# zalgo3/zfista

Hardware: AMD Instinct MI355X
Metric: fista_iterations_per_sec_n1e8_per_gpu_shard (higher is better)
Workload: dtype f64

## Files before the change

zfista_amd/_lib.py:

```python
from __future__ import annotations

import ctypes as C
import os
import subprocess

import numpy as np

_HERE = os.path.dirname(os.path.abspath(__file__))
CSRC = os.path.join(_HERE, "csrc")
LIB_PATH = os.environ.get("ZF_LIB_PATH") or os.path.join(CSRC, "libzfista_hip.so")

ZF_OK = 0
ZF_RUNNING, ZF_CONVERGED, ZF_MAXITER, ZF_BACKTRACK_FAILED = 0, 1, 2, 3
ZF_PROBLEM_DIAG_QUAD_L1, ZF_PROBLEM_LEAST_SQUARES_L1, ZF_PROBLEM_BLUR_HAAR_L1 = 1, 2, 3
ZF_PROBLEM_SPARSE_LS_L1 = 4
ZF_PROBLEM_LOGISTIC_L1, ZF_PROBLEM_SPARSE_LOGISTIC_L1 = 5, 6
ZF_MO_GENERIC, ZF_MO_JOS1, ZF_MO_FDS = 0, 1, 2
ZF_PACK_LEN, ZF_TRACE_COLS, ZF_RING = 8, 8, 1024
ZF_MAX_SUB_ITERS = 16
ZF_MAX_LAG = 2 * ZF_MAX_SUB_ITERS - 2
ZF_PEND_FLUSH = -1
TR_ERR, TR_F, TR_LR, TR_FUN, TR_TRIALS, TR_FX, TR_GX, TR_FY = range(8)
PK_FY, PK_DOT, PK_SS, PK_GX, PK_FX, PK_ERR = range(6)
PK_DF = 7
ZF_ACCEPT_REFERENCE, ZF_ACCEPT_RESOLVED, ZF_ACCEPT_REMAINDER = 0, 1, 2
ACCEPT_MODES = {"reference": ZF_ACCEPT_REFERENCE, "resolved": ZF_ACCEPT_RESOLVED, "remainder": ZF_ACCEPT_REMAINDER}


class HipUnavailable(RuntimeError):
    """The HIP engine cannot be used (library not built, or no GPU)."""


class ZfError(RuntimeError):
    """A libzfista_hip call returned a negative status."""


# ... 219 lines not shown
    lib = load()
    n = C.c_int(0)
    rc = lib.zf_device_count(C.byref(n))
    if rc != ZF_OK or n.value < 1:
        raise HipUnavailable(
            "no usable GPU: " + lib.zf_last_error().decode(errors="replace")
            + " - zfista_amd runs its solver arithmetic on MI355X only (no CPU fallback)."
        )
    return lib


ENV_SWITCHES = ("ZF_SPECULATE", "ZF_LS_SMALL", "ZF_GEMV_MFMA", "ZF_TILES_PER_WG", "ZF_SUB_ITERS",
                "ZF_COMM", "ZF_MO_COMM", "ZF_MO_LAUNCH_AHEAD", "ZF_MO_SPIN_LIMIT", "ZF_RCCL_LIB", "ZF_DUAL_SOLVER",
                "ZF_FORCE_SPLIT", "ZF_LIB_PATH", "ZF_BENCH_BACKEND",
                "ZF_RUNAHEAD", "ZF_RUNAHEAD_SPIN_LIMIT", "ZF_PASS_SEQ_START", "ZF_AHEAD",
                "ZF_AHEAD_UNSHARDED", "ZF_ACCEPT", "ZF_OP_SEPARABLE", "ZF_OP_FUSE_PROX", "ZF_OP_PERSIST", "ZF_RUNAHEAD_SHARDED")


def env_overrides() -> dict:
    return {k: os.environ[k] for k in ENV_SWITCHES if k in os.environ}


def ptr(a: np.ndarray) -> int:
    return a.ctypes.data
```

zfista_amd/csrc/zf_common.h:

```cpp
#pragma once
#include <hip/hip_runtime.h>
#include <stdint.h>
#include <stdio.h>
#include <string.h>

#include "../../include/zfista_hip.h"

extern thread_local char zf_errbuf[512];
static inline int zf_fail(int code, const char* fmt, const char* a = "", const char* b = "") {
    snprintf(zf_errbuf, sizeof(zf_errbuf), fmt, a, b);
    return code;
}
#define ZF_HIP(expr)                                                                   \
    do {                                                                               \
        hipError_t _e = (expr);                                                        \
        if (_e != hipSuccess) return zf_fail(ZF_ERR_HIP, "%s: %s", #expr, hipGetErrorString(_e)); \
    } while (0)
#define ZF_REQUIRE(cond, msg)                                  \
    do {                                                       \
        if (!(cond)) return zf_fail(ZF_ERR_ARG, "%s%s", msg);  \
    } while (0)

struct zf_env {
    bool speculate;
    int pass_seq_start;
    int sub_iters;
    bool runahead;
    int tiles_per_wg;
    unsigned runahead_spin;
    int runahead_sharded;
    bool ahead;
    bool ahead_unsharded;
    bool gemv_mfma;
    bool ls_small;
    bool op_separable;
    bool op_fuse_prox;
    bool op_persist;
    long long mo_spin_limit;
};
zf_env zf_env_read();

constexpr int ZF_BLOCK = 256;
constexpr int ZF_MAX_GRID = 2048;
constexpr int ZF_WAVES = ZF_BLOCK / 64;

static inline int zf_grid_for(int64_t items_per_thread_units) {
    int64_t blocks = (items_per_thread_units + ZF_BLOCK - 1) / ZF_BLOCK;
    if (blocks < 1) blocks = 1;
    if (blocks > ZF_MAX_GRID) blocks = ZF_MAX_GRID;
    return (int)blocks;
}

// ... 107 lines not shown
```

zfista_amd/csrc/zf_decide.h:

```cpp
#pragma once
#include <math.h>
#include <stddef.h>
#include <stdint.h>

#include "../../include/zfista_hip.h"

#if defined(__HIPCC__)
#define ZF_HD __host__ __device__
#else
#define ZF_HD
#endif

enum { ZF_PK_FY = 0, ZF_PK_DOT = 1, ZF_PK_SS = 2, ZF_PK_GX = 3, ZF_PK_FX = 4, ZF_PK_ERR = 5, ZF_PK_DF = 7 };
enum { ZF_TR_ERR = 0, ZF_TR_F = 1, ZF_TR_LR = 2, ZF_TR_FUN = 3, ZF_TR_TRIALS = 4,
       ZF_TR_FX = 5, ZF_TR_GX = 6, ZF_TR_FY = 7 };

ZF_HD inline void zf_reduce_packs(const double* packs, int world, int stride, double* out) {
    for (int k = 0; k < ZF_PACK_LEN; ++k) out[k] = packs[k];
    for (int r = 1; r < world; ++r) {
        const double* p = packs + (int64_t)r * stride;
        for (int k = 0; k < ZF_PACK_LEN; ++k) {
            if (k == ZF_PK_ERR) out[k] = (p[k] > out[k] || p[k] != p[k]) ? p[k] : out[k];
            else out[k] = out[k] + p[k];
        }
    }
}

ZF_HD inline void zf_free_bufs(int cur, int prev, int ring, int* first, int* second) {
    int f[2] = {-1, -1}, m = 0;
    if (ring >= 5) {
// ... 2 lines not shown
            if (i != prev) f[m++] = i;
        }
    } else {
        for (int i = 0; i < ring && m < 2; ++i)
            if (i != cur && i != prev) f[m++] = i;
    }
    *first = f[0];
    *second = (m > 1) ? f[1] : f[0];
}

ZF_HD inline int zf_fresh_len(const zf_control* c) {
    if (c->pend_status != 0) return 0;
    const int sub = c->sub_iters > 0 ? c->sub_iters : 1;
    const int64_t left = c->max_iter - c->nit;
    int64_t n = sub >= 16 ? sub / 2 : sub;
    if (c->lag == 0) {
        if (left >= 2 * (int64_t)sub || left == sub) return sub;
        n = left > sub ? (left + 1) / 2 : left;
    }
    const int64_t cap = (int64_t)(2 * sub - 1) - c->lag;
    if (n > cap) n = cap;
    if (n > left) n = left;
    if (n < 1) n = 1;
    return (int)n;
}

ZF_HD inline double zf_pack_stamp(const zf_control* c) {
    return (double)(((c->total_trials + 1) << 6) | ((int64_t)(c->lag & 31) << 1) | (c->pend_status != 0 ? 1 : 0));
}

typedef struct zf_trial_eval {
// ... 115 lines not shown
    const int sub = ctl->sub_iters > 0 ? ctl->sub_iters : 1;
    const int ring = ctl->ring_size > 0 ? ctl->ring_size : 3;
    const int stride = sub * ZF_PACK_LEN;
    const int lag = ctl->lag;
    zf_control c = *ctl;
    if (ctl->pend_status != 0) {
        if (lag > 0) zf_commit_chain(&c, ctl->cur, ctl->prev, ring, lag);
        c.lag = 0;
        if (c.pend_status > 0) c.status = c.pend_status;
        c.pend_status = 0;
        zf_resolve_beta(&c, beta_ring);
        zf_store_head(ctl, &c);
        return;
    }
    const int nf = zf_fresh_len(ctl);
    int accepted = 0;
    for (int j = 0; j < nf; ++j) {
        const int64_t before = c.nit;
        const double lr_used = c.lr;
        const bool go = zf_decide_step(&c, packs + j * ZF_PACK_LEN, trace, beta_ring, stride, pre ? pre + j : nullptr);
        if (c.nit > before) {
            if (lag + accepted < ZF_MAX_LAG) ctl->lag_lr[lag + accepted] = lr_used;
            accepted += 1;
        }
        if (!go) break;
    }
    if (accepted == nf) {
        zf_commit_chain(&c, ctl->cur, ctl->prev, ring, lag + nf);
        c.lag = 0;
    } else {
        c.lag = lag + accepted;
        if (c.status != ZF_RUNNING && c.lag > 0) {
            c.pend_status = c.status;
            c.status = ZF_RUNNING;
        }
    }
    zf_resolve_beta(&c, beta_ring);
    zf_store_head(ctl, &c);
}

#if defined(__HIPCC__)
__device__ __forceinline__ void zf_decide_pass_wave(zf_control* ctl, const double* packs,
// ... 16 lines not shown
```

zfista_amd/csrc/zf_kernels_step.h:

```cpp
#pragma once
#include <type_traits>

#include "zf_common.h"
#include "zf_decide.h"

constexpr int ZF_NPART = 6;

struct zf_elem_acc {
    double fy, dot, ss, l1, fx, mx;
};

template <bool NESTEROV, bool BOX, bool RES = false>
__device__ __forceinline__ double zf_elem_diag(double xk, double xo, double d, double c, double beta,
                                               double lr, double tau, double lo, double hi,
                                               zf_elem_acc& a) {
    double y = xk;
    if (NESTEROV) y = xk + beta * (xk - xo);
    const double r = y - c;
    const double grad = d * r;
    a.fy = __builtin_fma(grad, r, a.fy);
    const double v = y - lr * grad;
    double xn = zf_soft_threshold_nn(v, tau);
    if (BOX) xn = zf_clip(xn, lo, hi);
    const double dx = xn - y;
// ... 172 lines not shown
    int decide;
    double* trace;
    int pass_seq;
    int fb_on, fb_part, fb_len;
    unsigned long long* ra_word;
    unsigned* ra_flags;
    int ra_wait;
    int ra_need;
    unsigned ra_spin;
    zf_pass_head ra_head;
    unsigned* ra_stats;
    double head_stamp;
    int head_nf;
    int fin_grid;
    int accept_mode;
};

ZF_HD inline int zf_log_shape(int lag, int nf, int passes) { return (nf & 31) | ((lag & 31) << 5) | ((passes & 63) << 10); }

struct zf_finalize_args {
    const double* blk_part;
    int nblocks;
    int sub_iters;
    double* slice_part;
    unsigned* cnt;
    double scale[ZF_NPART];
    const double* f_y_ext;
    const double* f_x_ext;
    const double* r_ext;
    int contribute_f;
// ... 409 lines not shown
__device__ __forceinline__ double zf_readlane_f64(double v, int i) {
    const long long b = __double_as_longlong(v);
    const unsigned lo = (unsigned)__builtin_amdgcn_readlane((int)(unsigned)b, i);
    const unsigned hi = (unsigned)__builtin_amdgcn_readlane((int)(unsigned)(b >> 32), i);
    return __longlong_as_double((long long)(((unsigned long long)hi << 32) | lo));
}
__device__ __forceinline__ zf_pass_head zf_head_of(const zf_control* c) {
    zf_pass_head h;
    h.cur = c->cur;
    h.prev = c->prev;
    h.ring = c->ring_size;
    h.lr = c->lr;
    h.beta_next = c->beta_next;
    h.nit = c->nit;
    return h;
}

template <bool GRAD_INLINE, bool NESTEROV, bool BOX, bool NT, int S, int MODE, bool HIST, int SP = S, bool COH = false, bool RES = false>
__device__ __forceinline__ double zf_trial_body(const zf_step_args& A, double* lds, const zf_pass_head& HD, const int lag,
                                                const int nf, zf_d2* stage = nullptr) {
    constexpr bool FULL = (MODE == 0);
    static_assert(!RES || GRAD_INLINE, "resolved differences f(x+) - f(y): the separable problem");
    static_assert(!COH || (FULL && !HIST && GRAD_INLINE && SP >= 16 && ZF_S16_GLDS != 0),
                  "coherent iterate traffic: branch-free chains of a 16-chain solver through the DMA pipeline");
    constexpr bool GLDS = COH || zf_uses_glds<S, MODE, HIST, GRAD_INLINE, SP>();
    const unsigned tidx = threadIdx.x;
    constexpr bool FRESH_FULL = (MODE <= 1);
    const int cur = HD.cur;
    const int prev = HD.prev;
    const int ring = HD.ring;
// ... 276 lines not shown
                    o = a;
                    a = r;
                    if (HIST) A.hist[((nit + j + 1) % A.hist_cap) * A.hist_stride + e] = a;
                }
            }
            if constexpr (COH) {
                __hip_atomic_store(out_last + e, a, __ATOMIC_RELAXED, __HIP_MEMORY_SCOPE_AGENT);
                __hip_atomic_store(out_prev + e, o, __ATOMIC_RELAXED, __HIP_MEMORY_SCOPE_AGENT);
            } else {
                out_last[e] = a;
                if (S > 1 && (FRESH_FULL || ntr >= 2)) out_prev[e] = o;
            }
        }
    }

    constexpr int RS = S + (S > 1 ? (S & 1) : 0);
    constexpr int H = zf_chain_h(RS);
    constexpr int NQ = S * ZF_NPART;
    const int lane = tidx & 63, wave = tidx >> 6;
    double sums[5 * RS], maxs[RS];
#pragma unroll
    for (int j = 0; j < RS; ++j) {
        if (j < S) {
            sums[j * 5 + 0] = acc[j].fy;
            sums[j * 5 + 1] = acc[j].dot;
            sums[j * 5 + 2] = acc[j].ss;
            sums[j * 5 + 3] = acc[j].l1;
            sums[j * 5 + 4] = acc[j].fx;
            maxs[j] = acc[j].mx;
        } else {
#pragma unroll
            for (int k = 0; k < 5; ++k) sums[j * 5 + k] = 0.0;
            maxs[j] = 0.0;
        }
    }
    zf_wave_reduce_multi<5 * RS, H, false>(sums, lane);
    zf_wave_reduce_multi<RS, H, true>(maxs, lane);
    if ((lane & ((64 >> H) - 1)) == 0) {
#pragma unroll
        for (int q = 0; q < ((5 * RS) >> H); ++q) {
            const int idx = zf_wave_reduce_multi_index<5 * RS, H>(q, lane);
            if (idx / 5 < S) lds[wave * NQ + (idx / 5) * ZF_NPART + idx % 5] = sums[q];
        }
#pragma unroll
        for (int q = 0; q < (RS >> H); ++q) {
            const int tr = zf_wave_reduce_multi_index<RS, H>(q, lane);
            if (tr < S) lds[wave * NQ + tr * ZF_NPART + 5] = maxs[q];
        }
    }
    __syncthreads();
    double v = 0.0;
    if (tidx < NQ) {
        const int t = tidx;
        v = lds[t];
#pragma unroll
        for (int w = 1; w < ZF_WAVES; ++w) v = (t % ZF_NPART == 5) ? fmax(v, lds[w * NQ + t]) : v + lds[w * NQ + t];
    }
    return v;
}

template <int SP>
__device__ __forceinline__ void zf_pass_finish(const zf_step_args& A, const double v) {
    if (A.fin_mode == 0) {
        if (threadIdx.x < SP * ZF_NPART) A.blk_part[(int64_t)threadIdx.x * gridDim.x + blockIdx.x] = v;
// ... 147 lines not shown
    const int go = A.ra_wait == 0 ? 1 : __builtin_amdgcn_readfirstlane(s_go);
    if (go == 0) {
        if (b == 0 && threadIdx.x == 0) __hip_atomic_fetch_add(A.ra_stats + 1, 1u, __ATOMIC_RELAXED, __HIP_MEMORY_SCOPE_AGENT);
        return;
    }
    const bool run = go == 1;
    HD.beta_next = NESTEROV ? zf_uniform_f64(A.beta_ring[HD.nit % ZF_RING]) : 0.0;
    double v = 0.0;
    if (run) v = zf_trial_body<true, NESTEROV, BOX, NT, LEN, 0, false, S, true, RES>(A, lds, HD, 0, LEN, stage);
    zf_step_args T = A;
    T.ctl = A.ctl_rw;
    T.ctl_rw = &s_ctl;
    zf_pass_tail<S, true, LEN>(T, v);
}

template <bool GRAD_INLINE, bool BOX>
__global__ __launch_bounds__(ZF_BLOCK) void zf_eval_kernel(const double* __restrict__ x,
                                                           const double* __restrict__ d,
                                                           const double* __restrict__ c, double lo,
                                                           double hi, int64_t n, double* partials) {
    __shared__ double lds[ZF_WAVES * 3];
    double f = 0.0, l1 = 0.0, viol = 0.0;
    const int64_t stride = (int64_t)gridDim.x * ZF_BLOCK;
    for (int64_t i = (int64_t)blockIdx.x * ZF_BLOCK + threadIdx.x; i < n; i += stride) {
        const double xv = x[i];
        if (GRAD_INLINE) {
            const double r = xv - c[i];
            f += d[i] * (r * r);
        }
        l1 += fabs(xv);
// ... 35 lines not shown
```

zfista_amd/csrc/zf_solver.hip:

```cpp
#include <algorithm>
#include <cstring>
#include <map>
#include <mutex>
#include <new>
#include <tuple>
#include <vector>

#include "zf_common.h"
#include "zf_decide.h"
#include "zf_kernels_gemv.h"
#include "zf_kernels_ls_small.h"
#include "zf_kernels_op.h"
#include "zf_spmv.h"
#include "zf_kernels_loss.h"
#include "zf_kernels_step.h"
#include "zf_trial_launch.h"

thread_local char zf_errbuf[512] = "";

__global__ __launch_bounds__(ZF_BLOCK) void zf_sum_parts_kernel(const zf_control* ctl, const double* __restrict__ s_all,
                                                                int world, int64_t m, zf_ring3 sr, int slot) {
    int idx = 0;
    if (slot >= 0) {
        if (ctl->status != ZF_RUNNING) return;
// ... 199 lines not shown
    double* blk_part2 = nullptr;
    double* grp_part2 = nullptr;
    unsigned* fin_cnt2 = nullptr;
    double* pack2 = nullptr;
    int64_t ra_passes = 0, ra_ahead = 0;
    unsigned* ra_stats = nullptr;
    int64_t ra_timeouts = 0, ra_voids = 0, ah_voids = 0, second_voids = 0;
    bool ra_off = false;
    bool ah = false;
    bool ah_unsharded = false;
    hipEvent_t ah_evT[4] = {}, ah_evD[4] = {};
    int ah_run = 0;
    int ah_last_nf = 0;
    int run_mode = 0;
    int64_t ah_passes = 0;
    double* hist = nullptr;
    int64_t hist_cap = 0, hist_stride = 0;
};
constexpr int ZF_PASS_LOG = 4096;
constexpr size_t ZF_CTL_SLOT = (sizeof(zf_control) + 255) / 256 * 256;
constexpr size_t ZF_STATS_OFF = ZF_CTL_SLOT - 32;
static_assert(sizeof(zf_control) <= ZF_STATS_OFF, "the run-ahead counters live behind the control block, inside its slot");
constexpr size_t ZF_TRACE_BYTES = sizeof(double) * ZF_RING * ZF_TRACE_COLS;
constexpr size_t ZF_MAIL_BYTES = ZF_CTL_SLOT + ZF_TRACE_BYTES + sizeof(int) * ZF_PASS_LOG;

static int zf_tiles_for(int64_t ntiles);
constexpr bool ZF_AHEAD_UNSHARDED_DEFAULT = false;

zf_env zf_env_read() {
    zf_env v;
    const char* e;
    v.speculate = !((e = getenv("ZF_SPECULATE")) && atoi(e) == 0);
    v.pass_seq_start = (e = getenv("ZF_PASS_SEQ_START")) ? (int)std::min<long long>(std::max<long long>(atoll(e), 0), 0x7ffffff0LL) : 0;
    v.sub_iters = (e = getenv("ZF_SUB_ITERS")) ? atoi(e) : 0;
    v.runahead = !((e = getenv("ZF_RUNAHEAD")) && atoi(e) == 0);
    v.tiles_per_wg = (e = getenv("ZF_TILES_PER_WG")) ? std::max(1, atoi(e)) : 0;
    v.runahead_spin = (e = getenv("ZF_RUNAHEAD_SPIN_LIMIT")) ? (unsigned)strtoul(e, nullptr, 10) : 1u << 13;
    v.runahead_sharded = (e = getenv("ZF_RUNAHEAD_SHARDED")) ? (atoi(e) != 0 ? 1 : 0) : -1;
    v.ahead = !((e = getenv("ZF_AHEAD")) && atoi(e) == 0);
    v.ahead_unsharded = (e = getenv("ZF_AHEAD_UNSHARDED")) ? atoi(e) != 0 : ZF_AHEAD_UNSHARDED_DEFAULT;
    v.gemv_mfma = !((e = getenv("ZF_GEMV_MFMA")) && atoi(e) == 0);
    v.ls_small = !((e = getenv("ZF_LS_SMALL")) && atoi(e) == 0);
    v.op_separable = !((e = getenv("ZF_OP_SEPARABLE")) && atoi(e) == 0);
    v.op_fuse_prox = !((e = getenv("ZF_OP_FUSE_PROX")) && atoi(e) == 0);
    v.op_persist = !((e = getenv("ZF_OP_PERSIST")) && atoi(e) == 0);
    v.mo_spin_limit = (e = getenv("ZF_MO_SPIN_LIMIT")) ? atoll(e) : 0;
    return v;
}

static int zf_solver_free_all(zf_solver* s) {
    if (s->stream2) (void)hipStreamDestroy(s->stream2);
    if (s->stream3) (void)hipStreamDestroy(s->stream3);
    if (s->ra_join3) (void)hipEventDestroy(s->ra_join3);
    for (int k = 0; k < 4; ++k) {
        if (s->ah_evT[k]) (void)hipEventDestroy(s->ah_evT[k]);
        if (s->ah_evD[k]) (void)hipEventDestroy(s->ah_evD[k]);
    }
    if (s->ra_join) (void)hipEventDestroy(s->ra_join);
    if (s->ra_fork) (void)hipEventDestroy(s->ra_fork);
    void* ptrs[] = {s->sp_part_A, s->sp_part_At, s->op_buf, s->row_part, s->ls_cnt, s->blk_part, s->slice_part, s->fin_cnt, s->grp_part, s->xbuf, s->partials, s->ctl_trace, s->beta_ring,
                    s->ra_word, s->ra_flags, s->blk_part2, s->grp_part2, s->fin_cnt2, s->pack2,
                    s->own_packs ? s->pack_local : nullptr, s->own_packs ? s->pack_all : nullptr,
                    s->grad, s->sbuf, s->resid, s->slab, s->ls_scal,
                    s->own_svec ? s->s_part : nullptr, s->own_svec ? s->s_all : nullptr};
    for (void* p : ptrs)
        if (p) (void)hipFree(p);
    if (s->mail) (void)hipHostFree(s->mail);
    for (auto& e : s->ev_pool) {
        (void)hipEventDestroy(e.first);
        (void)hipEventDestroy(e.second);
    }
    for (auto& e : s->xev_pool) {
        (void)hipEventDestroy(e.first);
        (void)hipEventDestroy(e.second);
    }
    return ZF_OK;
// ... 218 lines not shown
        }
    }
    ZF_TRY(hipMalloc(&s->xbuf, sizeof(double) * s->ring * n_pad));
    for (int k = 0; k < s->ring; ++k) s->xb[k] = s->xbuf + k * n_pad;
    ZF_TRY(hipMalloc(&s->partials, sizeof(double) * ZF_NPART * ZF_MAX_GRID));
    {
        int64_t parts = std::max<int64_t>(s->max_grid, n / LS_SMALL_COLS + 1);
        if (desc->kind == ZF_PROBLEM_BLUR_HAAR_L1)
            parts = std::max<int64_t>(parts, zf_op_make_plan(desc->op_h, desc->op_w, (int)desc->op_k, false, false).grid);
        ZF_TRY(hipMalloc(&s->blk_part, sizeof(double) * ZF_NPART * s->sub * parts));
    }
    ZF_TRY(hipMalloc(&s->slice_part, sizeof(double) * ZF_NPART * s->sub * ZF_FIN_WGS));
    ZF_TRY(hipMalloc(&s->fin_cnt, sizeof(unsigned) * ZF_FIN_CNT_STRIDE * (ZF_FIN_GROUPS + 2)));
    ZF_TRY(hipMemsetAsync(s->fin_cnt, 0, sizeof(unsigned) * ZF_FIN_CNT_STRIDE * (ZF_FIN_GROUPS + 2), s->stream));
    ZF_TRY(hipMalloc(&s->grp_part, sizeof(double) * ZF_NPART * s->sub * ZF_FIN_GROUPS));
    ZF_TRY(hipMalloc(&s->ctl_trace, ZF_MAIL_BYTES));
    s->ctl = reinterpret_cast<zf_control*>(s->ctl_trace);
    s->trace = reinterpret_cast<double*>(s->ctl_trace + ZF_CTL_SLOT);
    s->pass_log = reinterpret_cast<int*>(s->ctl_trace + ZF_CTL_SLOT + ZF_TRACE_BYTES);
    s->ra_stats = reinterpret_cast<unsigned*>(s->ctl_trace + ZF_STATS_OFF);
    ZF_TRY(hipMemsetAsync(s->ctl_trace, 0, ZF_CTL_SLOT, s->stream));
    ZF_TRY(hipMemsetAsync(s->pass_log, 0xff, sizeof(int) * ZF_PASS_LOG, s->stream));
    ZF_TRY(hipHostMalloc(&s->mail, ZF_MAIL_BYTES, hipHostMallocDefault));
    ZF_TRY(hipMalloc(&s->beta_ring, sizeof(double) * ZF_RING));
    ZF_TRY(hipMalloc(&s->pack_local, sizeof(double) * ZF_PACK_LEN * s->sub));
    ZF_TRY(hipMalloc(&s->pack_all, sizeof(double) * ZF_PACK_LEN * s->sub * desc->world));
    ZF_TRY(hipMemsetAsync(s->trace, 0, sizeof(double) * ZF_RING * ZF_TRACE_COLS, s->stream));
    ZF_TRY(hipMemsetAsync(s->beta_ring, 0, sizeof(double) * ZF_RING, s->stream));
    ZF_TRY(hipMemsetAsync(s->pack_all, 0, sizeof(double) * ZF_PACK_LEN * s->sub * desc->world, s->stream));
    if (desc->kind == ZF_PROBLEM_BLUR_HAAR_L1) {
// ... 74 lines not shown

extern "C" int zf_solver_destroy(zf_solver* s) {
    if (!s) return ZF_OK;
    (void)hipStreamSynchronize(s->stream);
    zf_solver_free_all(s);
    delete s;
    return ZF_OK;
}

enum {
    ZF_K_FULL = 1,
    ZF_K_SHORT = 2,
    ZF_K_GENERAL = 4,
    ZF_K_MID = 8,
    ZF_K_FALLBACK = 16,
    ZF_K_ALL = ZF_K_FULL | ZF_K_SHORT | ZF_K_GENERAL,
};

static void zf_launch_trial_kernels(zf_solver* s, const zf_step_args& a, bool grad_inline) {
    const zf_trial_sel v = zf_sel_of(s);
    const int mask = s->part_mask;
    const int grid = s->grid;
    hipStream_t st = s->stream;
    if (!grad_inline) {
        if (s->hist) zf_launch_hist(v, false, 1, 0, grid, st, a);
        else zf_launch_vec(v, grid, st, a);
        return;
    }
    if (s->hist) {
        const int S = s->sub == 8 ? 8 : 1;
        if (mask & ZF_K_FULL) zf_launch_hist(v, true, S, 0, grid, st, a);
        if (S > 1 && (mask & ZF_K_SHORT)) zf_launch_hist(v, true, S, 1, grid, st, a);
        return;
    }
    if (s->sub >= 16) {
        if (mask & ZF_K_FULL) zf_launch_s16_full(v, grid, st, a);
        if (mask & ZF_K_SHORT) zf_launch_s16_short(v, grid, st, a);
        if (mask & ZF_K_MID) zf_launch_s16_mid(v, s->mid_len, grid, st, a);
        if (mask & ZF_K_GENERAL) zf_launch_s16_general(v, grid, st, a);
        if (mask & ZF_K_FALLBACK) {
            zf_step_args f = a;
            f.fb_on = 1;
            f.fb_part = s->fb_part;
            f.fb_len = s->fb_len;
            zf_launch_s16_general(v, grid, st, f);
        }
        return;
    }
    if (mask & ZF_K_FULL) zf_launch_chain(v, s->sub, 0, grid, st, a);
    if (s->sub > 1 && (mask & ZF_K_SHORT)) zf_launch_chain(v, s->sub, 1, grid, st, a);
// ... 109 lines not shown
        return ZF_K_ALL;
    zf_control& c = s->shadow;
    const int S = s->sub;
    const bool s16 = S >= 16;
    if (c.status != ZF_RUNNING) {
        if (!s16) return ZF_K_ALL;
        if (s->grid > ZF_SMALL_GRID) {
            s->fb_part = 1;
            s->fb_len = 0;
            return ZF_K_SHORT | ZF_K_FALLBACK;
        }
        s->fb_part = -1;
        return ZF_K_FALLBACK;
    }
    const int lag = c.lag;
    const int nf = zf_fresh_len(&c);
    int part = zf_pass_part(S, lag, nf);
    const zf_trial_sel v = zf_sel_of(s);
    if (part == 3 && !zf_have_s16_mid(v, nf)) part = 2;
    int mask = part == 3 ? ZF_K_MID : (1 << part);
    s->mid_len = nf;
    if (s->careful && s->steps_since_poll > 0) {
        const int64_t left = c.max_iter - c.nit;
        if (!s16) {
            mask = ZF_K_ALL;
        } else if (s->grid <= ZF_SMALL_GRID) {
            s->fb_part = -1;
            mask = ZF_K_FALLBACK;
        } else {
            if (left >= 2 * (int64_t)S) {
// ... 247 lines not shown
            if (cap < 0) cap = zf_runahead_capacity(zf_sel_of(s), nf_before);
            ra_ok = cap > 0 && s->grid <= cap;
        }
        const bool ah_ok = ah_can && !ra_ok && exact && ((s->part_mask == ZF_K_FULL && nf_before == s->sub) ||
                                                          (s->part_mask == ZF_K_MID && nf_before == s->mid_len));
        if (s->stream2 && a.pass_seq == 1 && !dry) {
            int rc = zf_ra_join(s);
            if (rc) return rc;
            ZF_HIP(hipMemsetAsync(s->ra_word, 0, 128, s->stream));
            ZF_HIP(hipMemsetAsync(s->ra_flags, 0, sizeof(unsigned) * (s->max_grid + 32), s->stream));
            ZF_HIP(hipEventRecord(s->ra_fork, s->stream));
            ZF_HIP(hipStreamWaitEvent(s->stream2, s->ra_fork, 0));
        }
        if (!dry) {
            s->steps_since_poll += 1;
            const int shapes = s->part_mask & (s->sub >= 16 ? 31 : s->sub > 1 ? 3 : 1);
            s->steps_issued += 1;
            s->kernels_issued += __builtin_popcount(shapes);
        }
        if (ra_ok) {
            int rc = zf_launch_runahead(s, a, before, nf_before, e0, e1);
            if (rc) return rc;
            if (s->comm && done_ahead) *done_ahead = true;
        } else if (ah_ok) {
            int rc = zf_launch_ahead(s, a, before, s->part_mask == ZF_K_FULL ? 0 : 3, nf_before, e0, e1);
            if (rc) return rc;
            if (done_ahead) *done_ahead = true;
        } else {
            if (s->stream2) {
                int rc = zf_ra_join(s);
                if (rc) return rc;
// ... 1185 lines not shown
```

zfista_amd/csrc/zf_trial_launch.h:

```cpp
#pragma once
#include "zf_kernels_step.h"

struct zf_trial_sel {
    bool nest, box;
    bool res = false;
};

void zf_launch_s16_full(const zf_trial_sel& v, int grid, hipStream_t st, const zf_step_args& a);
void zf_launch_s16_short(const zf_trial_sel& v, int grid, hipStream_t st, const zf_step_args& a);
void zf_launch_s16_general(const zf_trial_sel& v, int grid, hipStream_t st, const zf_step_args& a);
bool zf_launch_s16_mid(const zf_trial_sel& v, int len, int grid, hipStream_t st, const zf_step_args& a);
bool zf_have_s16_mid(const zf_trial_sel& v, int len);
void zf_launch_s16_ahead_full(const zf_trial_sel& v, int grid, hipStream_t st, const zf_step_args& a);
bool zf_launch_s16_ahead_mid(const zf_trial_sel& v, int len, int grid, hipStream_t st, const zf_step_args& a);
void zf_launch_s16_tail(hipStream_t st, const zf_step_args& a);
bool zf_launch_s16_runahead(const zf_trial_sel& v, int len, int grid, hipStream_t st, const zf_step_args& a);
int zf_runahead_capacity(const zf_trial_sel& v, int len);
template <bool N, bool B, bool NT, bool RES, int L>
inline int zf_ra_kernel_op(int grid, hipStream_t st, const zf_step_args& a) {
    if (grid > 0) {
        hipLaunchKernelGGL((zf_runahead_kernel<N, B, NT, RES, L>), dim3(grid), dim3(ZF_BLOCK), 0, st, a);
        return 1;
    }
    static int cached = -1;
    if (cached >= 0) return cached;
    int per_cu = 0, dev = 0;
    hipDeviceProp_t prop;
// ... 38 lines not shown
```

zfista_amd/proximal_gradient.py:

```python
from __future__ import annotations

import collections.abc as _abc
import ctypes as C
import time
from warnings import warn

import numpy as np
from scipy.optimize import OptimizeResult

from . import _lib
from .engine import DeviceSolver, momentum_factors
from .problems import match_native, match_native_multi

_MSG_OK = "Optimization terminated successfully"
_MSG_MAXITER = "Maximum number of iterations reached"
_MSG_BACKTRACK = "Backtracking failed to find a suitable stepsize."
_MSG_DEPRECATED = (
    "Using the deprecated option is not mathematically proven to converge. "
    "Please consider using the recommended condition instead."
)
class IterateHistory(_abc.Sequence):

    def __init__(self, x0, n, length, ring, cap, stride, host):
        self._x0, self._n, self._len = x0, n, length
# ... 239 lines not shown
        lo = 0
        if first == 0:
            betas[0] = 0.0
            lo = 1
        if count - lo > 0:
            vals, self._t_state = momentum_factors(count - lo, self.ratio, self._t_state)
            betas[lo:] = vals
        self.solver.set_beta(first, betas)
        self._beta_filled = upto

    def advance(self, steps):
        self.enqueue_only(steps)
        return self.collect()

    def enqueue_only(self, steps):
        steps = int(min(steps, (_lib.ZF_RING - 1 - _lib.ZF_MAX_LAG) // self.sub_iters))
        if getattr(self, "_hist", None) is not None:
            steps = int(min(steps, self._history_room()))
        self._fill_beta(self.nit_seen + steps * self.sub_iters + 1)
        self.solver.enqueue(steps)

    def set_max_iter(self, max_iter):
        self.solver.set_max_iter(int(max_iter))
        self.opts = dict(self.opts, max_iter=int(max_iter))
        ctl, _ = self.solver.poll()
        self.status = int(ctl.status)
        self._fill_beta(self.nit_seen + 1)

    def collect(self):
        ctl, trace = self.solver.poll()
        idx = np.arange(self.nit_seen, ctl.nit) % _lib.ZF_RING
# ... 466 lines not shown
```

Measured before the change: 11470.

## Fuse final 17-22 FISTA iterations into one two-stage tail kernel

When 17 to 22 iterations remain on a large diagonal-quadratic L1 problem, the host launches one fused kernel with 512-thread workgroups. The first half runs roughly half the remaining chain and hands its elements through LDS to the second half, which runs the rest, so the tail no longer needs two separate passes over the vector. The control logic gains a DUE/HELD state so the first pass's acceptance is held until the second pass decides, and separate partial and pack buffers are added for the second half. This adds new code paths, extra device buffers and a tighter ring budget in exchange for removing one full memory sweep and one launch at the end of each run.

Measured after the change: 11280. 1.7% lower.

```diff
diff --git a/zfista_amd/_lib.py b/zfista_amd/_lib.py
--- a/zfista_amd/_lib.py
+++ b/zfista_amd/_lib.py
@@ -20,6 +20,8 @@
 ZF_MAX_SUB_ITERS = 16
 ZF_MAX_LAG = 2 * ZF_MAX_SUB_ITERS - 2
 ZF_PEND_FLUSH = -1
+ZF_FT_DUE, ZF_FT_HELD = 1, 2
+ZF_FT_MIN_LEFT, ZF_FT_MAX_LEFT = 17, 22
 TR_ERR, TR_F, TR_LR, TR_FUN, TR_TRIALS, TR_FX, TR_GX, TR_FY = range(8)
 PK_FY, PK_DOT, PK_SS, PK_GX, PK_FX, PK_ERR = range(6)
 PK_DF = 7
@@ -269,7 +271,8 @@
                 "ZF_COMM", "ZF_MO_COMM", "ZF_MO_LAUNCH_AHEAD", "ZF_MO_SPIN_LIMIT", "ZF_RCCL_LIB", "ZF_DUAL_SOLVER",
                 "ZF_FORCE_SPLIT", "ZF_LIB_PATH", "ZF_BENCH_BACKEND",
                 "ZF_RUNAHEAD", "ZF_RUNAHEAD_SPIN_LIMIT", "ZF_PASS_SEQ_START", "ZF_AHEAD",
-                "ZF_AHEAD_UNSHARDED", "ZF_ACCEPT", "ZF_OP_SEPARABLE", "ZF_OP_FUSE_PROX", "ZF_OP_PERSIST", "ZF_RUNAHEAD_SHARDED")
+                "ZF_AHEAD_UNSHARDED", "ZF_ACCEPT", "ZF_OP_SEPARABLE", "ZF_OP_FUSE_PROX", "ZF_OP_PERSIST", "ZF_RUNAHEAD_SHARDED",
+                "ZF_FUSED_TAIL")
 
 
 def env_overrides() -> dict:
diff --git a/zfista_amd/csrc/zf_common.h b/zfista_amd/csrc/zf_common.h
--- a/zfista_amd/csrc/zf_common.h
+++ b/zfista_amd/csrc/zf_common.h
@@ -36,6 +36,7 @@
     bool op_separable;
     bool op_fuse_prox;
     bool op_persist;
+    int fused_tail;
     long long mo_spin_limit;
 };
 zf_env zf_env_read();
diff --git a/zfista_amd/csrc/zf_decide.h b/zfista_amd/csrc/zf_decide.h
--- a/zfista_amd/csrc/zf_decide.h
+++ b/zfista_amd/csrc/zf_decide.h
@@ -14,6 +14,9 @@
 enum { ZF_PK_FY = 0, ZF_PK_DOT = 1, ZF_PK_SS = 2, ZF_PK_GX = 3, ZF_PK_FX = 4, ZF_PK_ERR = 5, ZF_PK_DF = 7 };
 enum { ZF_TR_ERR = 0, ZF_TR_F = 1, ZF_TR_LR = 2, ZF_TR_FUN = 3, ZF_TR_TRIALS = 4,
        ZF_TR_FX = 5, ZF_TR_GX = 6, ZF_TR_FY = 7 };
+
+enum { ZF_FT_DUE = 1, ZF_FT_HELD = 2 };
+enum { ZF_FT_MIN_LEFT = 17, ZF_FT_MAX_LEFT = 22 };
 
 ZF_HD inline void zf_reduce_packs(const double* packs, int world, int stride, double* out) {
     for (int k = 0; k < ZF_PACK_LEN; ++k) out[k] = packs[k];
@@ -46,7 +49,9 @@
     const int sub = c->sub_iters > 0 ? c->sub_iters : 1;
     const int64_t left = c->max_iter - c->nit;
     int64_t n = sub >= 16 ? sub / 2 : sub;
-    if (c->lag == 0) {
+    if (c->reserved0 == ZF_FT_HELD) {
+        n = left;
+    } else if (c->lag == 0) {
         if (left >= 2 * (int64_t)sub || left == sub) return sub;
         n = left > sub ? (left + 1) / 2 : left;
     }
@@ -192,6 +197,8 @@
         return;
     }
     const int nf = zf_fresh_len(ctl);
+    const int mark = ctl->reserved0;
+    c.reserved0 = 0;
     int accepted = 0;
     for (int j = 0; j < nf; ++j) {
         const int64_t before = c.nit;
@@ -203,7 +210,10 @@
         }
         if (!go) break;
     }
-    if (accepted == nf) {
+    if (accepted == nf && mark == ZF_FT_DUE && c.status == ZF_RUNNING) {
+        c.lag = lag + nf;
+        c.reserved0 = ZF_FT_HELD;
+    } else if (accepted == nf && mark != ZF_FT_DUE) {
         zf_commit_chain(&c, ctl->cur, ctl->prev, ring, lag + nf);
         c.lag = 0;
     } else {
diff --git a/zfista_amd/csrc/zf_kernels_step.h b/zfista_amd/csrc/zf_kernels_step.h
--- a/zfista_amd/csrc/zf_kernels_step.h
+++ b/zfista_amd/csrc/zf_kernels_step.h
@@ -210,6 +210,9 @@
     int head_nf;
     int fin_grid;
     int accept_mode;
+    double* blk_part_b;
+    double* grp_part_b;
+    double* pack_b;
 };
 
 ZF_HD inline int zf_log_shape(int lag, int nf, int passes) { return (nf & 31) | ((lag & 31) << 5) | ((passes & 63) << 10); }
@@ -649,6 +652,43 @@
     h.beta_next = c->beta_next;
     h.nit = c->nit;
     return h;
+}
+
+template <int S>
+__device__ __forceinline__ void zf_chain_wave_rows(const zf_elem_acc (&acc)[S], double* lds, const int lane, const int wave) {
+    constexpr int RS = S + (S > 1 ? (S & 1) : 0);
+    constexpr int H = zf_chain_h(RS);
+    constexpr int NQ = S * ZF_NPART;
+    double sums[5 * RS], maxs[RS];
+#pragma unroll
+    for (int j = 0; j < RS; ++j) {
+        if (j < S) {
+            sums[j * 5 + 0] = acc[j].fy;
+            sums[j * 5 + 1] = acc[j].dot;
+            sums[j * 5 + 2] = acc[j].ss;
+            sums[j * 5 + 3] = acc[j].l1;
+            sums[j * 5 + 4] = acc[j].fx;
+            maxs[j] = acc[j].mx;
+        } else {
+#pragma unroll
+            for (int k = 0; k < 5; ++k) sums[j * 5 + k] = 0.0;
+            maxs[j] = 0.0;
+        }
+    }
+    zf_wave_reduce_multi<5 * RS, H, false>(sums, lane);
+    zf_wave_reduce_multi<RS, H, true>(maxs, lane);
+    if ((lane & ((64 >> H) - 1)) == 0) {
+#pragma unroll
+        for (int q = 0; q < ((5 * RS) >> H); ++q) {
+            const int idx = zf_wave_reduce_multi_index<5 * RS, H>(q, lane);
+            if (idx / 5 < S) lds[wave * NQ + (idx / 5) * ZF_NPART + idx % 5] = sums[q];
+        }
+#pragma unroll
+        for (int q = 0; q < (RS >> H); ++q) {
+            const int tr = zf_wave_reduce_multi_index<RS, H>(q, lane);
+            if (tr < S) lds[wave * NQ + tr * ZF_NPART + 5] = maxs[q];
+        }
+    }
 }
 
 template <bool GRAD_INLINE, bool NESTEROV, bool BOX, bool NT, int S, int MODE, bool HIST, int SP = S, bool COH = false, bool RES = false>
@@ -955,40 +995,8 @@
         }
     }
 
-    constexpr int RS = S + (S > 1 ? (S & 1) : 0);
-    constexpr int H = zf_chain_h(RS);
     constexpr int NQ = S * ZF_NPART;
-    const int lane = tidx & 63, wave = tidx >> 6;
-    double sums[5 * RS], maxs[RS];
-#pragma unroll
-    for (int j = 0; j < RS; ++j) {
-        if (j < S) {
-            sums[j * 5 + 0] = acc[j].fy;
-            sums[j * 5 + 1] = acc[j].dot;
-            sums[j * 5 + 2] = acc[j].ss;
-            sums[j * 5 + 3] = acc[j].l1;
-            sums[j * 5 + 4] = acc[j].fx;
-            maxs[j] = acc[j].mx;
-        } else {
-#pragma unroll
-            for (int k = 0; k < 5; ++k) sums[j * 5 + k] = 0.0;
-            maxs[j] = 0.0;
-        }
-    }
-    zf_wave_reduce_multi<5 * RS, H, false>(sums, lane);
-    zf_wave_reduce_multi<RS, H, true>(maxs, lane);
-    if ((lane & ((64 >> H) - 1)) == 0) {
-#pragma unroll
-        for (int q = 0; q < ((5 * RS) >> H); ++q) {
-            const int idx = zf_wave_reduce_multi_index<5 * RS, H>(q, lane);
-            if (idx / 5 < S) lds[wave * NQ + (idx / 5) * ZF_NPART + idx % 5] = sums[q];
-        }
-#pragma unroll
-        for (int q = 0; q < (RS >> H); ++q) {
-            const int tr = zf_wave_reduce_multi_index<RS, H>(q, lane);
-            if (tr < S) lds[wave * NQ + tr * ZF_NPART + 5] = maxs[q];
-        }
-    }
+    zf_chain_wave_rows<S>(acc, lds, tidx & 63, tidx >> 6);
     __syncthreads();
     double v = 0.0;
     if (tidx < NQ) {
@@ -1166,6 +1174,304 @@
     zf_pass_tail<S, true, LEN>(T, v);
 }
 
+constexpr int ZF_FT_THREADS = 2 * ZF_BLOCK;
+constexpr int ZF_FT_MAX_L = (ZF_FT_MAX_LEFT + 1) / 2;
+ZF_HD inline bool zf_fused_left(int64_t left) { return left >= ZF_FT_MIN_LEFT && left <= ZF_FT_MAX_LEFT; }
+
+__device__ __forceinline__ void zf_ft_barrier() {
+    asm volatile("s_waitcnt lgkmcnt(0)\n\ts_barrier" ::: "memory");
+}
+
+template <bool NESTEROV, bool RES, int L>
+__device__ __forceinline__ void zf_ft_chain2(zf_d2& a, zf_d2& o, const zf_d2 q, const zf_d2 cc, const double (&beta)[L], const double lr,
+                                             const double tau, zf_elem_acc (&acc)[L]) {
+#pragma unroll
+    for (int j = 0; j < L; ++j) {
+        zf_d2 r;
+        r.x = zf_elem_diag<NESTEROV, false, RES>(a.x, o.x, q.x, cc.x, beta[j], lr, tau, 0.0, 0.0, acc[j]);
+        r.y = zf_elem_diag<NESTEROV, false, RES>(a.y, o.y, q.y, cc.y, beta[j], lr, tau, 0.0, 0.0, acc[j]);
+        o = a;
+        a = r;
+    }
+    __builtin_amdgcn_sched_barrier(0);
+}
+template <bool NESTEROV, bool RES, int L>
+__device__ __forceinline__ void zf_ft_chain1(double& a, double& o, const double q, const double cc, const double (&beta)[L], const double lr,
+                                             const double tau, zf_elem_acc (&acc)[L]) {
+#pragma unroll
+    for (int j = 0; j < L; ++j) {
+        const double r = zf_elem_diag<NESTEROV, false, RES>(a, o, q, cc, beta[j], lr, tau, 0.0, 0.0, acc[j]);
+        o = a;
+        a = r;
+    }
+}
+
+template <int SP>
+__device__ __forceinline__ void zf_fused_pass_tail(const zf_step_args& A, const double v) {
+    constexpr int NQ = SP * ZF_NPART;
+    __shared__ int s_role;
+    __shared__ double s_tot[2 * NQ];
+    __shared__ double s_pack[ZF_MAX_SUB_ITERS * ZF_PACK_LEN];
+    __shared__ zf_trial_eval s_pre[ZF_MAX_SUB_ITERS];
+    __shared__ zf_control s_ctl;
+    const int tid = (int)threadIdx.x, half = tid / ZF_BLOCK, t = tid % ZF_BLOCK;
+    const int G = (int)gridDim.x, b = (int)blockIdx.x;
+    const int gsz = A.fin_gsz, ng = A.fin_ng;
+    const bool grouped = gsz > 1;
+    const bool is_max = (t % ZF_NPART == ZF_NPART - 1);
+    double* blk = half ? A.blk_part_b : A.blk_part;
+    double* grp = half ? A.grp_part_b : A.grp_part;
+    if (t < NQ) zf_publish(blk + (int64_t)b * NQ + t, v);
+    asm volatile("s_waitcnt vmcnt(0)" ::: "memory");
+    __syncthreads();
+    if (tid == 0) {
+        const int g = grouped ? b / gsz : 0;
+        unsigned* cnt = grouped ? A.fin_cnt + (1 + g) * ZF_FIN_CNT_STRIDE : A.fin_cnt;
+        int members = G;
+        if (grouped) members = (g + 1) * gsz <= G ? gsz : G - g * gsz;
+        const unsigned tk = __hip_atomic_fetch_add(cnt, 1u, __ATOMIC_RELAXED, __HIP_MEMORY_SCOPE_AGENT);
+        int role = 0;
+        if (tk == (unsigned)(members - 1)) {
+            __hip_atomic_store(cnt, 0u, __ATOMIC_RELAXED, __HIP_MEMORY_SCOPE_AGENT);
+            role = grouped ? 1 : 2;
+        }
+        asm volatile("s_waitcnt vmcnt(0)" ::: "memory");
+        s_role = role;
+    }
+    __syncthreads();
+    if (s_role == 0) return;
+    if (s_role == 1) {
+        const int g = b / gsz, b0 = g * gsz;
+        const int b1 = b0 + gsz <= G ? b0 + gsz : G;
+        if (t < NQ) zf_publish(grp + (int64_t)g * NQ + t, zf_sum_rows<NQ>(blk + (int64_t)b0 * NQ + t, b1 - b0, is_max));
+        asm volatile("s_waitcnt vmcnt(0)" ::: "memory");
+        __syncthreads();
+        if (tid == 0) {
+            const unsigned tk = __hip_atomic_fetch_add(A.fin_cnt, 1u, __ATOMIC_RELAXED, __HIP_MEMORY_SCOPE_AGENT);
+            const int last = (tk == (unsigned)(ng - 1));
+            if (last) __hip_atomic_store(A.fin_cnt, 0u, __ATOMIC_RELAXED, __HIP_MEMORY_SCOPE_AGENT);
+            asm volatile("s_waitcnt vmcnt(0)" ::: "memory");
+            s_role = last ? 2 : 0;
+        }
+        __syncthreads();
+        if (s_role != 2) return;
+    }
+    if (t < NQ) s_tot[half * NQ + t] = grouped ? zf_sum_rows<NQ>(grp + t, ng, is_max) : zf_sum_rows<NQ>(blk + t, G, is_max);
+    __syncthreads();
+    if (tid >= 64) return;
+    constexpr int CW = (int)(sizeof(zf_control) / 8);
+    static_assert(sizeof(zf_control) % 8 == 0 && CW <= 64, "one lane per word of the control block");
+    unsigned long long* gw = reinterpret_cast<unsigned long long*>(A.ctl_rw);
+    unsigned long long* lw = reinterpret_cast<unsigned long long*>(&s_ctl);
+    if (tid < CW) lw[tid] = gw[tid];
+    __builtin_amdgcn_wave_barrier();
+    if (tid == 0) s_ctl.reserved0 = ZF_FT_DUE;
+    __builtin_amdgcn_wave_barrier();
+    constexpr int SH = zf_chain_h(SP);
+    constexpr int LSTR = 64 >> SH;
+    const int trial = tid / LSTR;
+#pragma unroll 1
+    for (int h = 0; h < 2; ++h) {
+        if (h == 1 && __builtin_amdgcn_readfirstlane(s_ctl.reserved0) != ZF_FT_HELD) break;
+        const double* q = s_tot + h * NQ + trial * ZF_NPART;
+        double pk[ZF_PACK_LEN];
+        pk[ZF_PK_FY] = A.fin_scale_f * q[0];
+        pk[ZF_PK_DOT] = q[1];
+        pk[ZF_PK_SS] = q[2];
+        pk[ZF_PK_GX] = A.fin_scale_g * q[3];
+        pk[ZF_PK_FX] = A.fin_scale_f * q[4];
+        pk[ZF_PK_ERR] = q[5];
+        pk[6] = 0.0;
+        pk[7] = 0.0;
+        if (A.accept_mode != 0) {
+            pk[7] = pk[ZF_PK_FX];
+            pk[ZF_PK_FX] = pk[ZF_PK_FY] + pk[7];
+        }
+        double* pack = h ? A.pack_b : A.pack;
+        if (tid % LSTR == 0) {
+#pragma unroll
+            for (int k = 0; k < ZF_PACK_LEN; ++k) {
+                pack[trial * ZF_PACK_LEN + k] = pk[k];
+                s_pack[trial * ZF_PACK_LEN + k] = pk[k];
+            }
+        }
+        __builtin_amdgcn_wave_barrier();
+        zf_decide_pass_wave(&s_ctl, s_pack, pk, A.trace, A.beta_ring, tid, LSTR, s_pre);
+        __builtin_amdgcn_wave_barrier();
+    }
+    if (tid == 0) {
+        s_ctl.reserved0 = 0;
+        s_ctl.pass_seq = A.pass_seq;
+    }
+    __builtin_amdgcn_wave_barrier();
+    if (tid < CW) gw[tid] = lw[tid];
+}
+
+template <bool NESTEROV, bool RES, int LA, int LB>
+__global__ __launch_bounds__(ZF_FT_THREADS) void zf_fused_tail_kernel(zf_step_args A) {
+    constexpr int S = ZF_MAX_SUB;
+    static_assert(S == 16 && LA >= LB && LA - LB <= 1 && LA + LB >= ZF_FT_MIN_LEFT && LA + LB <= ZF_FT_MAX_LEFT && LA <= ZF_FT_MAX_L,
+                  "the two halves of a tail shared by two passes of a 16-chain solver");
+    constexpr int NST = ZF_GLDS_NST;
+    constexpr int NL = NESTEROV ? 4 : 3;
+    static_assert(NST == 3, "the counted waits of stage A are written for three DMA stages");
+    __shared__ zf_d2 stage[NST * ZF_GLDS_STAGE_UNITS];
+    __shared__ zf_d2 hand[2 * ZF_GLDS_STAGE_UNITS];
+    __shared__ double lds[2 * ZF_WAVES * ZF_FT_MAX_L * ZF_NPART];
+    const zf_control* c = A.ctl;
+    if (c->status != ZF_RUNNING || c->pass_seq == A.pass_seq) return;
+    if (c->lag != 0 || c->pend_status != 0 || c->reserved0 != 0 || c->max_iter - c->nit != LA + LB) return;
+    const zf_pass_head HD = zf_head_of(c);
+    const bool stage_b = __builtin_amdgcn_readfirstlane((int)threadIdx.x) >= ZF_BLOCK;
+    const unsigned tidx = threadIdx.x % ZF_BLOCK;
+    if (A.pass_log && blockIdx.x == 0 && threadIdx.x == 0) A.pass_log[A.pass_slot] = A.pass_tag | zf_log_shape(0, LA + LB, 0);
+    const double lr = HD.lr;
+    const double tau = A.lam * lr;
+    const int64_t nit = HD.nit;
+    int first, second;
+    zf_free_bufs(HD.cur, HD.prev, HD.ring, &first, &second);
+    const double* __restrict__ xk = A.xb[HD.cur];
+    const double* __restrict__ xo = A.xb[HD.prev];
+    double* __restrict__ out_last = A.xb[second];
+    double* __restrict__ out_prev = A.xb[first];
+    const double* __restrict__ p0 = A.p0;
+    const double* __restrict__ p1 = A.p1;
+    const int64_t n = A.n;
+    const int64_t n2 = n >> 1;
+    const int64_t G = gridDim.x;
+    const int full_tiles32 = (int)(n2 / ZF_TILE_UNITS), G32 = (int)gridDim.x, b32 = (int)blockIdx.x;
+    int my_tiles = 0;
+    for (int t = 0; t < A.tiles_per_wg; ++t)
+        if (t * G32 + b32 < full_tiles32) my_tiles = t + 1;
+    const int total = my_tiles * ZF_TILE_U;
+    auto unit_of = [&](int k) -> int64_t {
+        return ((int64_t)(k / ZF_TILE_U) * G + blockIdx.x) * ZF_TILE_UNITS + (k % ZF_TILE_U) * ZF_BLOCK + tidx;
+    };
+    const int64_t rem0 = (int64_t)full_tiles32 * ZF_TILE_UNITS * 2;
+    const int rem_trips = (rem0 != n && b32 == full_tiles32 % G32) ? (int)((n - rem0 + ZF_BLOCK - 1) / ZF_BLOCK) : 0;
+    double* hand1 = reinterpret_cast<double*>(hand);
+    const int lane = tidx & 63, wave = tidx >> 6;
+    if (!stage_b) {
+        double beta[LA];
+        beta[0] = NESTEROV ? HD.beta_next : 0.0;
+#pragma unroll
+        for (int j = 1; j < LA; ++j) beta[j] = NESTEROV ? A.beta_ring[(nit + j) % ZF_RING] : 0.0;
+        zf_elem_acc acc[LA];
+#pragma unroll
+        for (int j = 0; j < LA; ++j) acc[j] = {0.0, 0.0, 0.0, 0.0, 0.0, 0.0};
+        const zf_d2* __restrict__ xk2 = reinterpret_cast<const zf_d2*>(xk);
+        const zf_d2* __restrict__ xo2 = reinterpret_cast<const zf_d2*>(xo);
+        const zf_d2* __restrict__ p02 = reinterpret_cast<const zf_d2*>(p0);
+        const zf_d2* __restrict__ p12 = reinterpret_cast<const zf_d2*>(p1);
+        const unsigned lds0 = __builtin_amdgcn_readfirstlane((unsigned)(size_t)(zf_lds_ptr)stage + wave * 1024u);
+        auto issue = [&](int k) {
+            const int64_t i = unit_of(k);
+            const unsigned base = lds0 + (unsigned)(k % NST) * (ZF_GLDS_STAGE_UNITS * 16u);
+            zf_glds16<ZF_X_NT != 0>(xk2 + i, base);
+            if (NESTEROV) zf_glds16<ZF_X_NT != 0>(xo2 + i, base + ZF_BLOCK * 16u);
+            zf_glds16<true>(p02 + i, base + 2 * ZF_BLOCK * 16u);
+            zf_glds16<true>(p12 + i, base + 3 * ZF_BLOCK * 16u);
+        };
+#pragma unroll
+        for (int k = 0; k < NST - 1; ++k)
+            if (k < total) issue(k);
+        zf_wait_vm<0>();
+        int st = 0;
+        auto trip = [&](int k, auto more_c) {
+            constexpr bool MORE = decltype(more_c)::value;
+            const zf_d2* sp = stage + st * ZF_GLDS_STAGE_UNITS + tidx;
+            st = (st + 1 == NST) ? 0 : st + 1;
+            zf_d2 a = sp[0];
+            zf_d2 o = NESTEROV ? sp[ZF_BLOCK] : a;
+            const zf_d2 q = sp[2 * ZF_BLOCK];
+            const zf_d2 cc = sp[3 * ZF_BLOCK];
+            __builtin_amdgcn_sched_barrier(0);
+            if constexpr (MORE) issue(k + NST - 1);
+            zf_ft_chain2<NESTEROV, RES, LA>(a, o, q, cc, beta, lr, tau, acc);
+            zf_d2* hp = hand + (k & 1) * ZF_GLDS_STAGE_UNITS + tidx;
+            hp[0] = a;
+            hp[ZF_BLOCK] = o;
+            hp[2 * ZF_BLOCK] = q;
+            hp[3 * ZF_BLOCK] = cc;
+            if constexpr (MORE) zf_wait_vm<NL * (NST - 2)>();
+            else zf_wait_vm<0>();
+            zf_ft_barrier();
+        };
+        const int steady = total - (NST - 1);
+        int k = 0;
+#pragma unroll 1
+        for (; k < steady; ++k) trip(k, std::true_type{});
+#pragma unroll 1
+        for (; k < total; ++k) trip(k, std::false_type{});
+        zf_ft_barrier();
+        for (int r = 0; r < rem_trips; ++r) {
+            const int64_t e = rem0 + (int64_t)r * ZF_BLOCK + tidx;
+            if (e < n) {
+                double a = xk[e];
+                double o = NESTEROV ? xo[e] : a;
+                const double q = p0[e], cc = p1[e];
+                zf_ft_chain1<NESTEROV, RES, LA>(a, o, q, cc, beta, lr, tau, acc);
+                hand1[tidx] = a;
+                hand1[ZF_BLOCK + tidx] = o;
+                hand1[2 * ZF_BLOCK + tidx] = q;
+                hand1[3 * ZF_BLOCK + tidx] = cc;
+            }
+            zf_ft_barrier();
+            zf_ft_barrier();
+        }
+        zf_chain_wave_rows<LA>(acc, lds, lane, wave);
+    } else {
+        double beta[LB];
+#pragma unroll
+        for (int j = 0; j < LB; ++j) beta[j] = NESTEROV ? A.beta_ring[(nit + LA + j) % ZF_RING] : 0.0;
+        zf_elem_acc acc[LB];
+#pragma unroll
+        for (int j = 0; j < LB; ++j) acc[j] = {0.0, 0.0, 0.0, 0.0, 0.0, 0.0};
+        zf_ft_barrier();
+#pragma unroll 1
+        for (int k = 1; k <= total; ++k) {
+            {
+                const zf_d2* hp = hand + ((k - 1) & 1) * ZF_GLDS_STAGE_UNITS + tidx;
+                zf_d2 a = hp[0];
+                zf_d2 o = hp[ZF_BLOCK];
+                const zf_d2 q = hp[2 * ZF_BLOCK];
+                const zf_d2 cc = hp[3 * ZF_BLOCK];
+                __builtin_amdgcn_sched_barrier(0);
+                zf_ft_chain2<NESTEROV, RES, LB>(a, o, q, cc, beta, lr, tau, acc);
+                const int64_t i = unit_of(k - 1);
+                zf_st2<true>(reinterpret_cast<zf_d2*>(out_last) + i, a);
+                zf_st2<true>(reinterpret_cast<zf_d2*>(out_prev) + i, o);
+            }
+            zf_ft_barrier();
+        }
+        for (int r = 0; r < rem_trips; ++r) {
+            const int64_t e = rem0 + (int64_t)r * ZF_BLOCK + tidx;
+            zf_ft_barrier();
+            if (e < n) {
+                double a = hand1[tidx];
+                double o = hand1[ZF_BLOCK + tidx];
+                const double q = hand1[2 * ZF_BLOCK + tidx], cc = hand1[3 * ZF_BLOCK + tidx];
+                zf_ft_chain1<NESTEROV, RES, LB>(a, o, q, cc, beta, lr, tau, acc);
+                out_last[e] = a;
+                out_prev[e] = o;
+            }
+            zf_ft_barrier();
+        }
+        zf_chain_wave_rows<LB>(acc, lds + ZF_WAVES * ZF_FT_MAX_L * ZF_NPART, lane, wave);
+    }
+    __syncthreads();
+    const int NQS = (stage_b ? LB : LA) * ZF_NPART;
+    const double* row = lds + (stage_b ? ZF_WAVES * ZF_FT_MAX_L * ZF_NPART : 0);
+    double v = 0.0;
+    if ((int)tidx < NQS) {
+        const int t = (int)tidx;
+        v = row[t];
+#pragma unroll
+        for (int w = 1; w < ZF_WAVES; ++w) v = (t % ZF_NPART == 5) ? fmax(v, row[w * NQS + t]) : v + row[w * NQS + t];
+    }
+    zf_fused_pass_tail<S>(A, v);
+}
+
 template <bool GRAD_INLINE, bool BOX>
 __global__ __launch_bounds__(ZF_BLOCK) void zf_eval_kernel(const double* __restrict__ x,
                                                            const double* __restrict__ d,
diff --git a/zfista_amd/csrc/zf_solver.hip b/zfista_amd/csrc/zf_solver.hip
--- a/zfista_amd/csrc/zf_solver.hip
+++ b/zfista_amd/csrc/zf_solver.hip
@@ -237,6 +237,11 @@
     int ah_last_nf = 0;
     int run_mode = 0;
     int64_t ah_passes = 0;
+    bool fused = false;
+    int ft_left = 0;
+    double* ft_blk_part = nullptr;
+    double* ft_grp_part = nullptr;
+    double* ft_pack = nullptr;
     double* hist = nullptr;
     int64_t hist_cap = 0, hist_stride = 0;
 };
@@ -249,6 +254,7 @@
 
 static int zf_tiles_for(int64_t ntiles);
 constexpr bool ZF_AHEAD_UNSHARDED_DEFAULT = false;
+constexpr int64_t ZF_FT_MIN_N = 25000000;
 
 zf_env zf_env_read() {
     zf_env v;
@@ -268,6 +274,7 @@
     v.op_fuse_prox = !((e = getenv("ZF_OP_FUSE_PROX")) && atoi(e) == 0);
     v.op_persist = !((e = getenv("ZF_OP_PERSIST")) && atoi(e) == 0);
     v.mo_spin_limit = (e = getenv("ZF_MO_SPIN_LIMIT")) ? atoll(e) : 0;
+    v.fused_tail = (e = getenv("ZF_FUSED_TAIL")) ? (strcmp(e, "force") == 0 ? 2 : atoi(e) != 0 ? 1 : 0) : 1;
     return v;
 }
 
@@ -282,7 +289,7 @@
     if (s->ra_join) (void)hipEventDestroy(s->ra_join);
     if (s->ra_fork) (void)hipEventDestroy(s->ra_fork);
     void* ptrs[] = {s->sp_part_A, s->sp_part_At, s->op_buf, s->row_part, s->ls_cnt, s->blk_part, s->slice_part, s->fin_cnt, s->grp_part, s->xbuf, s->partials, s->ctl_trace, s->beta_ring,
-                    s->ra_word, s->ra_flags, s->blk_part2, s->grp_part2, s->fin_cnt2, s->pack2,
+                    s->ra_word, s->ra_flags, s->blk_part2, s->grp_part2, s->fin_cnt2, s->pack2, s->ft_blk_part, s->ft_grp_part, s->ft_pack,
                     s->own_packs ? s->pack_local : nullptr, s->own_packs ? s->pack_all : nullptr,
                     s->grad, s->sbuf, s->resid, s->slab, s->ls_scal,
                     s->own_svec ? s->s_part : nullptr, s->own_svec ? s->s_all : nullptr};
@@ -531,6 +538,13 @@
     ZF_TRY(hipMalloc(&s->fin_cnt, sizeof(unsigned) * ZF_FIN_CNT_STRIDE * (ZF_FIN_GROUPS + 2)));
     ZF_TRY(hipMemsetAsync(s->fin_cnt, 0, sizeof(unsigned) * ZF_FIN_CNT_STRIDE * (ZF_FIN_GROUPS + 2), s->stream));
     ZF_TRY(hipMalloc(&s->grp_part, sizeof(double) * ZF_NPART * s->sub * ZF_FIN_GROUPS));
+    s->fused = s->env.fused_tail != 0 && desc->kind == ZF_PROBLEM_DIAG_QUAD_L1 && s->sub == 16 && desc->world == 1 && !s->box &&
+               (s->env.fused_tail == 2 || n >= ZF_FT_MIN_N);
+    if (s->fused) {
+        ZF_TRY(hipMalloc(&s->ft_blk_part, sizeof(double) * ZF_NPART * s->sub * s->max_grid));
+        ZF_TRY(hipMalloc(&s->ft_grp_part, sizeof(double) * ZF_NPART * s->sub * ZF_FIN_GROUPS));
+        ZF_TRY(hipMalloc(&s->ft_pack, sizeof(double) * ZF_PACK_LEN * s->sub));
+    }
     ZF_TRY(hipMalloc(&s->ctl_trace, ZF_MAIL_BYTES));
     s->ctl = reinterpret_cast<zf_control*>(s->ctl_trace);
     s->trace = reinterpret_cast<double*>(s->ctl_trace + ZF_CTL_SLOT);
@@ -635,6 +649,7 @@
     ZF_K_GENERAL = 4,
     ZF_K_MID = 8,
     ZF_K_FALLBACK = 16,
+    ZF_K_FUSED = 32,
     ZF_K_ALL = ZF_K_FULL | ZF_K_SHORT | ZF_K_GENERAL,
 };
 
@@ -655,6 +670,13 @@
         return;
     }
     if (s->sub >= 16) {
+        if (mask & ZF_K_FUSED) {
+            zf_step_args f = a;
+            f.blk_part_b = s->ft_blk_part;
+            f.grp_part_b = s->ft_grp_part;
+            f.pack_b = s->ft_pack;
+            zf_launch_s16_fused_tail(v, s->ft_left, grid, st, f);
+        }
         if (mask & ZF_K_FULL) zf_launch_s16_full(v, grid, st, a);
         if (mask & ZF_K_SHORT) zf_launch_s16_short(v, grid, st, a);
         if (mask & ZF_K_MID) zf_launch_s16_mid(v, s->mid_len, grid, st, a);
@@ -794,6 +816,16 @@
         return ZF_K_FALLBACK;
     }
     const int lag = c.lag;
+    if (s->fused && !s->hist && !s->comm && lag == 0 && c.pend_status == 0 && zf_fused_left(c.max_iter - c.nit) &&
+        !(s->careful && s->steps_since_poll > 0)) {
+        const int left = (int)(c.max_iter - c.nit);
+        s->ft_left = left;
+        c.nit += left;
+        c.total_trials += left;
+        zf_commit_chain(&c, c.cur, c.prev, c.ring_size > 0 ? c.ring_size : 3, left);
+        c.status = ZF_MAXITER;
+        return ZF_K_FUSED;
+    }
     const int nf = zf_fresh_len(&c);
     int part = zf_pass_part(S, lag, nf);
     const zf_trial_sel v = zf_sel_of(s);
@@ -1071,7 +1103,7 @@
         }
         if (!dry) {
             s->steps_since_poll += 1;
-            const int shapes = s->part_mask & (s->sub >= 16 ? 31 : s->sub > 1 ? 3 : 1);
+            const int shapes = s->part_mask & (s->sub >= 16 ? 63 : s->sub > 1 ? 3 : 1);
             s->steps_issued += 1;
             s->kernels_issued += __builtin_popcount(shapes);
         }
diff --git a/zfista_amd/csrc/zf_trial_launch.h b/zfista_amd/csrc/zf_trial_launch.h
--- a/zfista_amd/csrc/zf_trial_launch.h
+++ b/zfista_amd/csrc/zf_trial_launch.h
@@ -11,6 +11,7 @@
 void zf_launch_s16_general(const zf_trial_sel& v, int grid, hipStream_t st, const zf_step_args& a);
 bool zf_launch_s16_mid(const zf_trial_sel& v, int len, int grid, hipStream_t st, const zf_step_args& a);
 bool zf_have_s16_mid(const zf_trial_sel& v, int len);
+bool zf_launch_s16_fused_tail(const zf_trial_sel& v, int left, int grid, hipStream_t st, const zf_step_args& a);
 void zf_launch_s16_ahead_full(const zf_trial_sel& v, int grid, hipStream_t st, const zf_step_args& a);
 bool zf_launch_s16_ahead_mid(const zf_trial_sel& v, int len, int grid, hipStream_t st, const zf_step_args& a);
 void zf_launch_s16_tail(hipStream_t st, const zf_step_args& a);
diff --git a/zfista_amd/csrc/zf_trial_s16_fused_tail.hip b/zfista_amd/csrc/zf_trial_s16_fused_tail.hip
--- /dev/null
+++ b/zfista_amd/csrc/zf_trial_s16_fused_tail.hip
@@ -0,0 +1,25 @@
+#include "zf_trial_launch.h"
+
+template <bool N, bool R>
+static bool zf_launch_fused_tail_nr(int left, int grid, hipStream_t st, const zf_step_args& a) {
+#define FT(LEFT)                                                                                                               \
+    case LEFT:                                                                                                                 \
+        hipLaunchKernelGGL((zf_fused_tail_kernel<N, R, (LEFT + 1) / 2, LEFT / 2>), dim3(grid), dim3(ZF_FT_THREADS), 0, st, a); \
+        return true;
+    switch (left) {
+        FT(17)
+        FT(18)
+        FT(19)
+        FT(20)
+        FT(21)
+        FT(22)
+    }
+#undef FT
+    return false;
+}
+
+bool zf_launch_s16_fused_tail(const zf_trial_sel& v, int left, int grid, hipStream_t st, const zf_step_args& a) {
+    if (v.box) return false;
+    if (v.res) return v.nest ? zf_launch_fused_tail_nr<true, true>(left, grid, st, a) : zf_launch_fused_tail_nr<false, true>(left, grid, st, a);
+    return v.nest ? zf_launch_fused_tail_nr<true, false>(left, grid, st, a) : zf_launch_fused_tail_nr<false, false>(left, grid, st, a);
+}
diff --git a/zfista_amd/proximal_gradient.py b/zfista_amd/proximal_gradient.py
--- a/zfista_amd/proximal_gradient.py
+++ b/zfista_amd/proximal_gradient.py
@@ -277,7 +277,7 @@
         return self.collect()
 
     def enqueue_only(self, steps):
-        steps = int(min(steps, (_lib.ZF_RING - 1 - _lib.ZF_MAX_LAG) // self.sub_iters))
+        steps = int(min(steps, (_lib.ZF_RING - 1 - _lib.ZF_MAX_LAG - (_lib.ZF_FT_MAX_LEFT - _lib.ZF_MAX_SUB_ITERS)) // self.sub_iters))
         if getattr(self, "_hist", None) is not None:
             steps = int(min(steps, self._history_room()))
         self._fill_beta(self.nit_seen + steps * self.sub_iters + 1)
```
